# xUhEngwAng/I2V-Adapter-Unofficial

Measured on AMD Instinct MI355X. Metric: denoising steps/sec @ 16fx512x512 SD1.5+I2V-Adapter, higher is better.
Workload: dtype f16

## Files before the change

i2v-adapter-unofficial_amd/csrc/attention.hip:

```cpp
#include <cstdlib>
#include <type_traits>

#include "common.h"

namespace {

constexpr float DEFER_THR = 8.0f;

__device__ __forceinline__ float fast_exp2(float x) { return __builtin_amdgcn_exp2f(x); }
__device__ __forceinline__ float max3(float a, float b, float c) { return fmaxf(fmaxf(a, b), c); }

__device__ __forceinline__ float xor16_max(float x) { return lane_xor16_max(x); }
__device__ __forceinline__ float xor32_max(float x) { return lane_xor32_max(x); }

__device__ __forceinline__ uint32_t pack_rtz(float a, float b) {
  const auto h = __builtin_amdgcn_cvt_pkrtz(a, b);
  return __builtin_bit_cast(uint32_t, h);
}
__device__ __forceinline__ uint32_t pack_rn(float a, float b) {
  const f16x2 h = {(f16)a, (f16)b};
  return __builtin_bit_cast(uint32_t, h);
}

#ifndef I2V_ATTN_XCD_REMAP
#define I2V_ATTN_XCD_REMAP 1
#endif
#ifndef I2V_ATTN_OCC_D80
#define I2V_ATTN_OCC_D80 1
#endif
template <int DQK, int DPV, int QT, int KVT, bool SPARE, bool WALK = false>
__global__ __launch_bounds__(256)
__attribute__((amdgpu_waves_per_eu(DQK == 64 && DPV == 48 && QT == 2 && KVT == 64 && !WALK ? 4 : (DQK == 96 && DPV == 80 && !WALK ? I2V_ATTN_OCC_D80 : 1))))
void attn_kernel(const i2v_attn_params p, const float scale_log2, const int qbw_arg) {
  const int qbw = WALK ? qbw_arg : 1;
  constexpr int KS = DQK + 8;
  constexpr int VS = KVT + 8;
  constexpr int KSTEPS = DQK / 32;
  constexpr int DT = DPV / 16;
  constexpr int NKT = KVT / 16;
  constexpr int NS2 = KVT / 32;
  constexpr int KCH = DQK / 8;
  constexpr int VCH = KVT / 8;
  static_assert((KVT * KCH) % 256 == 0, "the K tile must be whole 16-byte chunks per thread");
  constexpr int NKC = (KVT * KCH) / 256;
  constexpr int NVC = (DPV * VCH + 255) / 256;
  constexpr int NSTG = WALK ? 1 : 2;
  __shared__ __attribute__((aligned(16))) f16 sKb[NSTG][KVT * KS];
  __shared__ __attribute__((aligned(16))) f16 sVb[NSTG][DPV * VS];

  const int tid = threadIdx.x, lane = tid & 63, wave = tid >> 6;
  const int g = lane >> 4, l15 = lane & 15;
  int qb = blockIdx.x, h = blockIdx.y, bq = blockIdx.z;
  {
    const int nqb = gridDim.x, pairs = gridDim.y * gridDim.z;
    if (I2V_ATTN_XCD_REMAP && p.lk <= 128 && (nqb * (int)gridDim.z) % 8 == 0) {
      const int lin = blockIdx.x + nqb * (blockIdx.y + gridDim.y * blockIdx.z);
      const int xcd = lin & 7, slot = lin >> 3;
      h = slot % (int)gridDim.y;
      const int unit = (slot / (int)gridDim.y) * 8 + xcd;
      qb = unit % nqb;
      bq = unit / nqb;
    } else if (I2V_ATTN_XCD_REMAP && pairs % 8 == 0) {
      const int lin = blockIdx.x + nqb * (blockIdx.y + gridDim.y * blockIdx.z);
      const int xcd = lin & 7, slot = lin >> 3;
      const int pair = (slot / nqb) * 8 + xcd;
      qb = slot % nqb;
      h = pair % (int)gridDim.y;
      bq = pair / (int)gridDim.y;
    }
  }
  const int bkv = bq / p.kv_group;
  const int d = p.head_dim, lq = p.lq, lk = p.lk;
  const int qb_first = qb * qbw;
  int q0 = qb_first * (64 * QT) + wave * (16 * QT);

  const f16* __restrict__ Q = reinterpret_cast<const f16*>(p.q) + (int64_t)bq * p.q_batch_stride + h * d;
  const f16* __restrict__ Kg = reinterpret_cast<const f16*>(p.k) + (int64_t)bkv * p.k_batch_stride + h * d;
  const f16* __restrict__ Vg =
      reinterpret_cast<const f16*>(p.vt) + (int64_t)bkv * p.vt_batch_stride + (int64_t)h * d * p.vt_row_stride;

  f16x8 qf[QT][KSTEPS];
  f32x4 o[DT][QT];
  f32x4 negm[QT];
  float lrow[QT];
  f16x8 qraw[QT][KSTEPS];
  auto fetch_q = [&](int q0f) {
#pragma unroll
    for (int qt = 0; qt < QT; ++qt) {
      const int row = q0f + qt * 16 + l15;
#pragma unroll
      for (int s = 0; s < KSTEPS; ++s) {
        const int dd = 32 * s + 8 * g;
        qraw[qt][s] = (row < lq && dd < d) ? ld_global_16B(Q + (int64_t)row * p.q_row_stride + dd) : zero8();
      }
    }
  };
  auto load_q = [&]() {
#pragma unroll
    for (int qt = 0; qt < QT; ++qt) {
#pragma unroll
      for (int s = 0; s < KSTEPS; ++s) {
        f16x8 v = qraw[qt][s];
#pragma unroll
        for (int e = 0; e < 8; ++e) v[e] = (f16)((float)v[e] * scale_log2);
        qf[qt][s] = v;
      }
    }
#pragma unroll
    for (int i = 0; i < DT; ++i)
#pragma unroll
      for (int j = 0; j < QT; ++j) o[i][j] = f32x4{0.f, 0.f, 0.f, 0.f};
#pragma unroll
    for (int j = 0; j < QT; ++j) {
      negm[j] = f32x4{0.f, 0.f, 0.f, 0.f};
      lrow[j] = 0.f;
    }
  };
  fetch_q(q0);

  constexpr int OOB = 0x40000000;
  f16x8 rk[NKC], rv[NVC];
  int k_off[NKC], v_off[NVC], k_lds[NKC], v_lds[NVC];
  const auto k_rsrc = __builtin_amdgcn_make_buffer_rsrc(
      const_cast<f16*>(Kg), 0, (int)(((int64_t)(lk - 1) * p.k_row_stride + d) * 2), 0x00020000);
  const auto v_rsrc = __builtin_amdgcn_make_buffer_rsrc(
      const_cast<f16*>(Vg), 0, (int)(((int64_t)(d - 1) * p.vt_row_stride + ((lk + 7) & ~7)) * 2), 0x00020000);
#pragma unroll
  for (int i = 0; i < NKC; ++i) {
    const int id = tid + 256 * i;
    const int row = id / KCH, c = id - row * KCH;
    k_off[i] = 8 * c < d ? (int)((row * p.k_row_stride + 8 * c) * 2) : OOB;
    const int lrow = (row & ~28) | ((row & 4) << 2) | ((row & 24) >> 1);
    k_lds[i] = lrow * KS + 8 * c;
  }
#pragma unroll
  for (int i = 0; i < NVC; ++i) {
    const int id = tid + 256 * i;
    const int row = id / VCH, c = id - row * VCH;
    v_off[i] = row < d ? (int)((row * p.vt_row_stride + 8 * c) * 2) : OOB;
    const bool real = row < DPV && !(SPARE && row == d);
    v_lds[i] = real ? row * VS + 8 * c : (tid % DPV) * VS + KVT;
  }
  if (SPARE && tid < NSTG * VCH) {
    f16x8 ones;
#pragma unroll
    for (int e = 0; e < 8; ++e) ones[e] = (f16)1.f;
    *reinterpret_cast<f16x8*>(&sVb[tid / VCH][d * VS + 8 * (tid % VCH)]) = ones;
  }
  const int k_tile_bytes = (int)(KVT * p.k_row_stride * 2);

  auto issue = [&](int t) {
    const int ks = t * k_tile_bytes, vs = t * (KVT * 2);
#pragma unroll
    for (int i = 0; i < NKC; ++i)
      rk[i] = __builtin_bit_cast(f16x8, __builtin_amdgcn_raw_buffer_load_b128(k_rsrc, k_off[i], ks, 0));
#pragma unroll
    for (int i = 0; i < NVC; ++i)
      rv[i] = __builtin_bit_cast(f16x8, __builtin_amdgcn_raw_buffer_load_b128(v_rsrc, v_off[i], vs, 0));
  };
  auto mask_tail_v = [&](int t) {
#pragma unroll
    for (int i = 0; i < NVC; ++i) {
      const int key0 = t * KVT + 8 * ((tid + 256 * i) % VCH);
#pragma unroll
      for (int e = 0; e < 8; ++e)
        if (key0 + e >= lk) rv[i][e] = (f16)0.f;
    }
  };
  auto commit = [&](int stage) {
    f16* sK = sKb[stage];
    f16* sV = sVb[stage];
#pragma unroll
    for (int i = 0; i < NKC; ++i) *reinterpret_cast<f16x8*>(&sK[k_lds[i]]) = rk[i];
#pragma unroll
    for (int i = 0; i < NVC; ++i) *reinterpret_cast<f16x8*>(&sV[v_lds[i]]) = rv[i];
  };

  const int ntiles = (lk + KVT - 1) / KVT;
  const bool partial = (lk % KVT) != 0;
  issue(0);
  if (ntiles == 1 && partial) mask_tail_v(0);
  commit(0);
  __syncthreads();

  auto process = [&](auto tail_c, auto more_c, const int t) {
    constexpr bool TAIL = decltype(tail_c)::value;
    constexpr bool more = decltype(more_c)::value;
    if (more) issue(t + 1);
    const f16* sK = sKb[t & 1];
    const f16* sV = sVb[t & 1];

    f32x4 sacc[NKT][QT];
#ifdef I2V_SETPRIO
    __builtin_amdgcn_s_setprio(1);
#endif
#pragma unroll
    for (int kt = 0; kt < NKT; ++kt) {
      const int krow = 16 * kt + l15;
#pragma unroll
      for (int s = 0; s < KSTEPS; ++s) {
        const f16x8 kf = *reinterpret_cast<const f16x8*>(&sK[krow * KS + 32 * s + 8 * g]);
#pragma unroll
        for (int j = 0; j < QT; ++j) sacc[kt][j] = mfma16x16x32(kf, qf[j][s], s == 0 ? negm[j] : sacc[kt][j]);
      }
    }

#ifdef I2V_SETPRIO
    __builtin_amdgcn_s_setprio(0);
#endif
    const int key_base = t * KVT;
    const bool first = t == 0;
    f16x8 pf[QT][NS2];
#pragma unroll
    for (int j = 0; j < QT; ++j) {
      float sv[NKT][4];
#pragma unroll
      for (int kt = 0; kt < NKT; ++kt)
#pragma unroll
        for (int r = 0; r < 4; ++r) {
          float v = sacc[kt][j][r];
          if (TAIL) {
            const int key = key_base + 32 * (kt >> 1) + 8 * g + 4 * (kt & 1) + r;
            if (key >= lk) v = -INFINITY;
          }
          sv[kt][r] = v;
        }
      float red[4 * NKT];
#pragma unroll
      for (int kt = 0; kt < NKT; ++kt)
#pragma unroll
        for (int r = 0; r < 4; ++r) red[4 * kt + r] = sv[kt][r];
      {
        int n = 4 * NKT;
#pragma unroll
        for (int level = 0; level < 5 && n > 1; ++level) {
          int m = 0;
#pragma unroll
          for (int i = 0; i + 2 < n; i += 3) red[m++] = max3(red[i], red[i + 1], red[i + 2]);
          if (n % 3 == 2) {
            red[m] = fmaxf(red[n - 2], red[n - 1]);
            ++m;
          } else if (n % 3 == 1) {
            red[m] = red[n - 1];
            ++m;
          }
          n = m;
        }
      }
      float mx = red[0];
      if (__any(first || mx > DEFER_THR)) {
        mx = xor16_max(mx);
        mx = xor32_max(mx);
        const float dlt = first ? mx : fmaxf(mx, 0.f);
        const float alpha = first ? 1.0f : fast_exp2(-dlt);
#pragma unroll
        for (int r = 0; r < 4; ++r) negm[j][r] -= dlt;
#pragma unroll
        for (int kt = 0; kt < NKT; ++kt)
#pragma unroll
          for (int r = 0; r < 4; ++r) sv[kt][r] -= dlt;
#pragma unroll
        for (int i = 0; i < DT; ++i)
#pragma unroll
          for (int r = 0; r < 4; ++r) o[i][j][r] *= alpha;
        if (!SPARE) lrow[j] *= alpha;
      }
      float ls = 0.f;
#pragma unroll
      for (int kt = 0; kt < NKT; ++kt)
#pragma unroll
        for (int r = 0; r < 4; ++r) {
          sv[kt][r] = fast_exp2(sv[kt][r]);
          if (!SPARE) ls += sv[kt][r];
        }
      if (!SPARE) lrow[j] += ls;
#pragma unroll
      for (int s2 = 0; s2 < NS2; ++s2) {
        u32x4 w;
        if (SPARE) {
          w[0] = pack_rtz(sv[2 * s2][0], sv[2 * s2][1]);
          w[1] = pack_rtz(sv[2 * s2][2], sv[2 * s2][3]);
          w[2] = pack_rtz(sv[2 * s2 + 1][0], sv[2 * s2 + 1][1]);
          w[3] = pack_rtz(sv[2 * s2 + 1][2], sv[2 * s2 + 1][3]);
        } else {
          w[0] = pack_rn(sv[2 * s2][0], sv[2 * s2][1]);
          w[1] = pack_rn(sv[2 * s2][2], sv[2 * s2][3]);
          w[2] = pack_rn(sv[2 * s2 + 1][0], sv[2 * s2 + 1][1]);
          w[3] = pack_rn(sv[2 * s2 + 1][2], sv[2 * s2 + 1][3]);
        }
        pf[j][s2] = __builtin_bit_cast(f16x8, w);
      }
    }

#ifdef I2V_SETPRIO
    __builtin_amdgcn_s_setprio(1);
#endif
#pragma unroll
    for (int s2 = 0; s2 < NS2; ++s2)
#pragma unroll
      for (int i = 0; i < DT; ++i) {
        const f16x8 vf = *reinterpret_cast<const f16x8*>(&sV[(i * 16 + l15) * VS + 32 * s2 + 8 * g]);
#pragma unroll
        for (int j = 0; j < QT; ++j) o[i][j] = mfma16x16x32(vf, pf[j][s2], o[i][j]);
      }

#ifdef I2V_SETPRIO
    __builtin_amdgcn_s_setprio(0);
#endif
    if (more) {
      if (partial && t + 2 == ntiles) mask_tail_v(t + 1);
      commit((t + 1) & 1);
      __syncthreads();
    }
  };

  for (int qi = 0; qi < qbw; ++qi) {
    if (WALK) {
      if ((qb_first + qi) * (64 * QT) >= lq) break;
      q0 = (qb_first + qi) * (64 * QT) + wave * (16 * QT);
    }
    load_q();
    if (WALK && qi + 1 < qbw) fetch_q(q0 + 64 * QT);
    for (int t = 0; t + 1 < ntiles; ++t) process(std::false_type{}, std::true_type{}, t);
    if (partial)
      process(std::true_type{}, std::false_type{}, ntiles - 1);
    else
      process(std::false_type{}, std::false_type{}, ntiles - 1);

    f16* __restrict__ O = reinterpret_cast<f16*>(p.o) + (int64_t)bq * p.o_batch_stride + h * d;
#pragma unroll
    for (int j = 0; j < QT; ++j) {
      float lt;
      if (SPARE) {
        float cand = 0.f;
#pragma unroll
        for (int i = 0; i < DT; ++i)
#pragma unroll
          for (int r = 0; r < 4; ++r)
            if (i == (d >> 4) && r == (d & 3)) cand = o[i][j][r];
        lt = __shfl(cand, (((d & 15) >> 2) << 4) | l15, 64);
      } else {
        lt = lrow[j];
        lt += __shfl_xor(lt, 16, 64);
        lt += __shfl_xor(lt, 32, 64);
      }
      const float inv = 1.0f / lt;
      const int row = q0 + j * 16 + l15;
      if (row >= lq) continue;
      if (p.lse != nullptr && g == 0)
        p.lse[((int64_t)bq * p.heads + h) * lq + row] = __builtin_amdgcn_logf(lt) - negm[j][0];
#pragma unroll
      for (int i = 0; i < DT; ++i) {
        const int dd = i * 16 + 4 * g;
        if (dd >= d) continue;
        f16* dst = O + (int64_t)row * p.o_row_stride + dd;
        f16x4 ov;
        if (p.accumulate) {
          const f16x4 prev = *reinterpret_cast<const f16x4*>(dst);
#pragma unroll
          for (int r = 0; r < 4; ++r) ov[r] = (f16)((float)prev[r] + p.acc_scale * o[i][j][r] * inv);
        } else {
#pragma unroll
          for (int r = 0; r < 4; ++r) ov[r] = (f16)(o[i][j][r] * inv);
        }
        *reinterpret_cast<f16x4*>(dst) = ov;
      }
    }
  }
}

inline bool al(const void* p, uintptr_t a) { return (reinterpret_cast<uintptr_t>(p) % a) == 0; }

template <int DQK, int DPV, bool SPARE>
int launch_q(const i2v_attn_params& p, hipStream_t s) {
  const float scale_log2 = p.scale * 1.4426950408889634f;
  int qt = 1;
  if (p.lq >= 128 && (DQK <= 96 || DQK == 160)) qt = 2;
  static const int qt_env = getenv("I2V_ATTN_QT") ? atoi(getenv("I2V_ATTN_QT")) : 0;
  static const int kvt_env = getenv("I2V_ATTN_KVT") ? atoi(getenv("I2V_ATTN_KVT")) : 0;
  if (qt_env == 1 || qt_env == 2) qt = qt_env;
  int kvt = 64;
  if (DQK == 64 && p.lk > 64 && p.lk <= 96) kvt = 96;
  if (kvt_env == 64 || (kvt_env == 128 && DQK <= 64) || (kvt_env == 96 && DQK == 64)) kvt = kvt_env;
  const dim3 block(256);
  const int nqb = (int)i2v_cdiv(p.lq, 64 * qt);
  static const int walk_off = getenv("I2V_ATTN_WALK") ? (atoi(getenv("I2V_ATTN_WALK")) == 0) : 0;
  int qbw = 1;
  if (!walk_off && p.lk <= kvt) {
    const int64_t wgs = (int64_t)nqb * p.heads * p.batch_q;
    qbw = (int)(wgs / 1024);
    if (qbw > 8) qbw = 8;
    if (qbw > nqb) qbw = nqb;
    if (qbw < 1) qbw = 1;
  }
  const bool walk = qbw > 1;
  const dim3 grid((unsigned)i2v_cdiv(nqb, qbw), (unsigned)p.heads, (unsigned)p.batch_q);
#define I2V_ATTN_LAUNCH(QTV, KVTV)                                                                                       \
  do {                                                                                                                   \
    if (walk)                                                                                                            \
      hipLaunchKernelGGL((attn_kernel<DQK, DPV, QTV, KVTV, SPARE, true>), grid, block, 0, s, p, scale_log2, qbw);        \
    else                                                                                                                 \
      hipLaunchKernelGGL((attn_kernel<DQK, DPV, QTV, KVTV, SPARE, false>), grid, block, 0, s, p, scale_log2, 1);         \
  } while (0)
  if constexpr (DQK == 64) {
    if (kvt == 96) {
      if (qt == 2) I2V_ATTN_LAUNCH(2, 96); else I2V_ATTN_LAUNCH(1, 96);
      return i2v_check_launch("i2v_attention_f16");
    }
  }
  if constexpr (DQK <= 64) {
    if (kvt == 128) {
      if (qt == 2) I2V_ATTN_LAUNCH(2, 128); else I2V_ATTN_LAUNCH(1, 128);
      return i2v_check_launch("i2v_attention_f16");
    }
  }
  if (qt == 2) I2V_ATTN_LAUNCH(2, 64); else I2V_ATTN_LAUNCH(1, 64);
#undef I2V_ATTN_LAUNCH
  return i2v_check_launch("i2v_attention_f16");
}

template <int DQK, int DPV>
int launch_d(const i2v_attn_params& p, hipStream_t s) {
  return p.head_dim < DPV ? launch_q<DQK, DPV, true>(p, s) : launch_q<DQK, DPV, false>(p, s);
}

}

#ifdef I2V_VARIANTS
int i2v_attention32_try(const i2v_attn_params& p, hipStream_t s);
int i2v_attention_pipe_try(const i2v_attn_params& p, hipStream_t s);
#endif

extern "C" int i2v_attention_f16(const i2v_attn_params* pp, i2v_stream_t stream) {
  I2V_CHECK_ARG(pp != nullptr, "i2v_attention_f16: null params");
  const i2v_attn_params& p = *pp;
  I2V_CHECK_ARG(p.q && p.k && p.vt && p.o, "i2v_attention_f16: null pointer");
  I2V_CHECK_ARG(p.batch_q > 0 && p.kv_group > 0 && p.batch_q % p.kv_group == 0,
                "i2v_attention_f16: batch_q (%d) must be a positive multiple of kv_group (%d)", p.batch_q, p.kv_group);
  I2V_CHECK_ARG(p.heads > 0 && p.lq > 0 && p.lk > 0, "i2v_attention_f16: heads, lq, lk must be positive");
  I2V_CHECK_ARG(!(p.lse != nullptr && p.accumulate), "i2v_attention_f16: lse output is not combined with accumulate");
  I2V_CHECK_ARG(p.head_dim > 0 && p.head_dim % 8 == 0 && p.head_dim <= 160,
                "i2v_attention_f16: head_dim (%d) must be a multiple of 8 and <= 160", p.head_dim);
  I2V_CHECK_ARG(p.q_row_stride % 8 == 0 && p.k_row_stride % 8 == 0 && p.q_batch_stride % 8 == 0 &&
                    p.k_batch_stride % 8 == 0,
                "i2v_attention_f16: q / k strides must be multiples of 8 elements");
  I2V_CHECK_ARG(p.vt_row_stride % 8 == 0 && p.vt_batch_stride % 8 == 0 && p.vt_row_stride >= ((p.lk + 7) / 8) * 8,
                "i2v_attention_f16: vt_row_stride must be a multiple of 8 and >= lk rounded up to 8");
  I2V_CHECK_ARG(p.o_row_stride % 4 == 0 && p.o_batch_stride % 4 == 0, "i2v_attention_f16: o strides must be multiples of 4");
  I2V_CHECK_ARG(al(p.q, 16) && al(p.k, 16) && al(p.vt, 16) && al(p.o, 8), "i2v_attention_f16: pointer alignment");
  I2V_CHECK_ARG(p.heads <= 65535 && p.batch_q <= 65535, "i2v_attention_f16: heads / batch_q exceed the grid limits");
  I2V_CHECK_ARG(p.k_row_stride > 0 && ((int64_t)p.lk + 128) * p.k_row_stride * 2 < (1ll << 30) &&
                    p.vt_row_stride > 0 && ((int64_t)p.head_dim * p.vt_row_stride + 256) * 2 < (1ll << 30),
                "i2v_attention_f16: one (batch, head) slice of K / V^T must span less than 1 GiB");
  hipStream_t s = reinterpret_cast<hipStream_t>(stream);
  const int d = p.head_dim;
  if (d <= 16) return launch_d<32, 16>(p, s);
  if (d <= 32) return launch_d<32, 32>(p, s);
#ifdef I2V_VARIANTS
  if (d > 32 && d < 48) {
    const int rc = i2v_attention_pipe_try(p, s);
    if (rc != 0) return rc < 0 ? rc : I2V_OK;
  }
  if (d > 32 && d <= 48) {
    const int rc = i2v_attention32_try(p, s);
    if (rc != 0) return rc < 0 ? rc : I2V_OK;
  }
#endif
  if (d <= 48) return launch_d<64, 48>(p, s);
  if (d <= 64) return launch_d<64, 64>(p, s);
  if (d <= 80) return launch_d<96, 80>(p, s);
  if (d <= 96) return launch_d<96, 96>(p, s);
  if (d <= 128) return launch_d<128, 128>(p, s);
  return launch_d<160, 160>(p, s);
}
```

Measured before the change: 20.99.

## Add max-free attention path fixing max from diagonal tile, with fallback redo

Adds a MAXFREE attention variant. It computes the row max once from a first tile (the diagonal tile when lq==lk) and then skips all later max tracking and rescaling. Row sums are accumulated with an MFMA against a ones vector instead of scalar adds. If any final row sum overflows a threshold, the block redoes the standard online-softmax walk, which costs extra work in rare cases and adds a shared-memory flag and a barrier. The variant is on by default for selected head-dim classes via an env var and also changes the occupancy hint.

```diff
diff --git a/i2v-adapter-unofficial_amd/csrc/attention.hip b/i2v-adapter-unofficial_amd/csrc/attention.hip
--- a/i2v-adapter-unofficial_amd/csrc/attention.hip
+++ b/i2v-adapter-unofficial_amd/csrc/attention.hip
@@ -28,11 +28,12 @@
 #ifndef I2V_ATTN_OCC_D80
 #define I2V_ATTN_OCC_D80 1
 #endif
-template <int DQK, int DPV, int QT, int KVT, bool SPARE, bool WALK = false>
+template <int DQK, int DPV, int QT, int KVT, bool SPARE, bool WALK = false, bool MAXFREE = false>
 __global__ __launch_bounds__(256)
-__attribute__((amdgpu_waves_per_eu(DQK == 64 && DPV == 48 && QT == 2 && KVT == 64 && !WALK ? 4 : (DQK == 96 && DPV == 80 && !WALK ? I2V_ATTN_OCC_D80 : 1))))
-void attn_kernel(const i2v_attn_params p, const float scale_log2, const int qbw_arg) {
-  const int qbw = WALK ? qbw_arg : 1;
+__attribute__((amdgpu_waves_per_eu(DQK == 64 && DPV == 48 && QT == 2 && KVT == 64 && !WALK ? 4 : (DQK == 96 && DPV == 80 && !WALK ? (MAXFREE && QT == 2 ? 2 : I2V_ATTN_OCC_D80) : 1))))
+void attn_kernel(const i2v_attn_params p, const float scale_log2, const int aux) {
+  static_assert(!(WALK && MAXFREE), "the single-tile walk has no later tiles");
+  const int qbw = WALK ? aux : 1;
   constexpr int KS = DQK + 8;
   constexpr int VS = KVT + 8;
   constexpr int KSTEPS = DQK / 32;
@@ -83,6 +84,8 @@
   f32x4 o[DT][QT];
   f32x4 negm[QT];
   float lrow[QT];
+  f32x4 lacc[QT];
+  bool l_in_mfma = false;
   f16x8 qraw[QT][KSTEPS];
   auto fetch_q = [&](int q0f) {
 #pragma unroll
@@ -106,6 +109,8 @@
         qf[qt][s] = v;
       }
     }
+  };
+  auto reset_acc = [&]() {
 #pragma unroll
     for (int i = 0; i < DT; ++i)
 #pragma unroll
@@ -114,6 +119,7 @@
     for (int j = 0; j < QT; ++j) {
       negm[j] = f32x4{0.f, 0.f, 0.f, 0.f};
       lrow[j] = 0.f;
+      lacc[j] = f32x4{0.f, 0.f, 0.f, 0.f};
     }
   };
   fetch_q(q0);
@@ -178,17 +184,28 @@
 
   const int ntiles = (lk + KVT - 1) / KVT;
   const bool partial = (lk % KVT) != 0;
-  issue(0);
+  __shared__ int s_redo;
+  const bool fast = MAXFREE && ntiles > 1;
+  const int nfull = partial ? ntiles - 1 : ntiles;
+  int t_start = 0;
+  if (fast && lq == lk && p.kv_group == 1) {
+    t_start = (qb * (64 * QT)) / KVT;
+    if (t_start >= nfull) t_start = nfull - 1;
+  }
+  if (MAXFREE && tid == 0) s_redo = 0;
+  issue(t_start);
   if (ntiles == 1 && partial) mask_tail_v(0);
   commit(0);
   __syncthreads();
 
-  auto process = [&](auto tail_c, auto more_c, const int t) {
+  auto process = [&](auto tail_c, auto more_c, auto mode_c, const int t, const int tn, const int stage) {
     constexpr bool TAIL = decltype(tail_c)::value;
     constexpr bool more = decltype(more_c)::value;
-    if (more) issue(t + 1);
-    const f16* sK = sKb[t & 1];
-    const f16* sV = sVb[t & 1];
+    constexpr int MODE = decltype(mode_c)::value;
+    if (more) issue(tn);
+    if constexpr (MODE != 0) __builtin_amdgcn_sched_barrier(0);
+    const f16* sK = sKb[stage];
+    const f16* sV = sVb[stage];
 
     f32x4 sacc[NKT][QT];
 #ifdef I2V_SETPRIO
@@ -225,6 +242,7 @@
           }
           sv[kt][r] = v;
         }
+      if constexpr (MODE != 2) {
       float red[4 * NKT];
 #pragma unroll
       for (int kt = 0; kt < NKT; ++kt)
@@ -248,7 +266,16 @@
         }
       }
       float mx = red[0];
-      if (__any(first || mx > DEFER_THR)) {
+      if constexpr (MODE == 1) {
+        mx = xor16_max(mx);
+        mx = xor32_max(mx);
+#pragma unroll
+        for (int r = 0; r < 4; ++r) negm[j][r] = -mx;
+#pragma unroll
+        for (int kt = 0; kt < NKT; ++kt)
+#pragma unroll
+          for (int r = 0; r < 4; ++r) sv[kt][r] -= mx;
+      } else if (__any(first || mx > DEFER_THR)) {
         mx = xor16_max(mx);
         mx = xor32_max(mx);
         const float dlt = first ? mx : fmaxf(mx, 0.f);
@@ -265,15 +292,16 @@
           for (int r = 0; r < 4; ++r) o[i][j][r] *= alpha;
         if (!SPARE) lrow[j] *= alpha;
       }
+      }
       float ls = 0.f;
 #pragma unroll
       for (int kt = 0; kt < NKT; ++kt)
 #pragma unroll
         for (int r = 0; r < 4; ++r) {
           sv[kt][r] = fast_exp2(sv[kt][r]);
-          if (!SPARE) ls += sv[kt][r];
-        }
-      if (!SPARE) lrow[j] += ls;
+          if (!SPARE && MODE == 0) ls += sv[kt][r];
+        }
+      if (!SPARE && MODE == 0) lrow[j] += ls;
 #pragma unroll
       for (int s2 = 0; s2 < NS2; ++s2) {
         u32x4 w;
@@ -303,15 +331,46 @@
 #pragma unroll
         for (int j = 0; j < QT; ++j) o[i][j] = mfma16x16x32(vf, pf[j][s2], o[i][j]);
       }
+    if constexpr (!SPARE && MODE != 0) {
+      f16x8 ones;
+#pragma unroll
+      for (int e = 0; e < 8; ++e) ones[e] = (f16)1.f;
+#pragma unroll
+      for (int s2 = 0; s2 < NS2; ++s2)
+#pragma unroll
+        for (int j = 0; j < QT; ++j) lacc[j] = mfma16x16x32(ones, pf[j][s2], lacc[j]);
+    }
 
 #ifdef I2V_SETPRIO
     __builtin_amdgcn_s_setprio(0);
 #endif
     if (more) {
-      if (partial && t + 2 == ntiles) mask_tail_v(t + 1);
-      commit((t + 1) & 1);
+      if (partial && tn + 1 == ntiles) mask_tail_v(tn);
+      commit(stage ^ 1);
       __syncthreads();
     }
+  };
+  [[maybe_unused]] constexpr std::integral_constant<int, 0> mode_defer{};
+  [[maybe_unused]] constexpr std::integral_constant<int, 1> mode_first{};
+  [[maybe_unused]] constexpr std::integral_constant<int, 2> mode_free{};
+  auto row_sum = [&](const int j) {
+    float lt;
+    if (SPARE) {
+      float cand = 0.f;
+#pragma unroll
+      for (int i = 0; i < DT; ++i)
+#pragma unroll
+        for (int r = 0; r < 4; ++r)
+          if (i == (d >> 4) && r == (d & 3)) cand = o[i][j][r];
+      lt = __shfl(cand, (((d & 15) >> 2) << 4) | l15, 64);
+    } else if (MAXFREE && l_in_mfma) {
+      lt = lacc[j][0];
+    } else {
+      lt = lrow[j];
+      lt += __shfl_xor(lt, 16, 64);
+      lt += __shfl_xor(lt, 32, 64);
+    }
+    return lt;
   };
 
   for (int qi = 0; qi < qbw; ++qi) {
@@ -320,30 +379,52 @@
       q0 = (qb_first + qi) * (64 * QT) + wave * (16 * QT);
     }
     load_q();
+    reset_acc();
     if (WALK && qi + 1 < qbw) fetch_q(q0 + 64 * QT);
-    for (int t = 0; t + 1 < ntiles; ++t) process(std::false_type{}, std::true_type{}, t);
-    if (partial)
-      process(std::true_type{}, std::false_type{}, ntiles - 1);
-    else
-      process(std::false_type{}, std::false_type{}, ntiles - 1);
+    bool defer_walk = true;
+    if constexpr (MAXFREE) {
+      if (fast) {
+        auto next_tile = [&](const int i) { return i + 1 < nfull ? (i < t_start ? i : i + 1) : nfull; };
+        l_in_mfma = !SPARE;
+        int t = t_start, tn = next_tile(0);
+        process(std::false_type{}, std::true_type{}, mode_first, t, tn, 0);
+        t = tn;
+        for (int i = 1; i + 1 < ntiles; ++i) {
+          tn = next_tile(i);
+          process(std::false_type{}, std::true_type{}, mode_free, t, tn, i & 1);
+          t = tn;
+        }
+        if (partial)
+          process(std::true_type{}, std::false_type{}, mode_free, t, 0, (ntiles - 1) & 1);
+        else
+          process(std::false_type{}, std::false_type{}, mode_free, t, 0, (ntiles - 1) & 1);
+        bool bad = aux != 0;
+#pragma unroll
+        for (int j = 0; j < QT; ++j) bad |= (__float_as_uint(row_sum(j)) & 0x7fffffffu) >= 0x47000000u;
+        if (bad) s_redo = 1;
+        __syncthreads();
+        defer_walk = s_redo != 0;
+        if (defer_walk) {
+          l_in_mfma = false;
+          reset_acc();
+          issue(0);
+          commit(0);
+          __syncthreads();
+        }
+      }
+    }
+    if (defer_walk) {
+      for (int t = 0; t + 1 < ntiles; ++t) process(std::false_type{}, std::true_type{}, mode_defer, t, t + 1, t & 1);
+      if (partial)
+        process(std::true_type{}, std::false_type{}, mode_defer, ntiles - 1, 0, (ntiles - 1) & 1);
+      else
+        process(std::false_type{}, std::false_type{}, mode_defer, ntiles - 1, 0, (ntiles - 1) & 1);
+    }
 
     f16* __restrict__ O = reinterpret_cast<f16*>(p.o) + (int64_t)bq * p.o_batch_stride + h * d;
 #pragma unroll
     for (int j = 0; j < QT; ++j) {
-      float lt;
-      if (SPARE) {
-        float cand = 0.f;
-#pragma unroll
-        for (int i = 0; i < DT; ++i)
-#pragma unroll
-          for (int r = 0; r < 4; ++r)
-            if (i == (d >> 4) && r == (d & 3)) cand = o[i][j][r];
-        lt = __shfl(cand, (((d & 15) >> 2) << 4) | l15, 64);
-      } else {
-        lt = lrow[j];
-        lt += __shfl_xor(lt, 16, 64);
-        lt += __shfl_xor(lt, 32, 64);
-      }
+      const float lt = row_sum(j);
       const float inv = 1.0f / lt;
       const int row = q0 + j * 16 + l15;
       if (row >= lq) continue;
@@ -411,6 +492,17 @@
   if constexpr (DQK <= 64) {
     if (kvt == 128) {
       if (qt == 2) I2V_ATTN_LAUNCH(2, 128); else I2V_ATTN_LAUNCH(1, 128);
+      return i2v_check_launch("i2v_attention_f16");
+    }
+  }
+  static const int maxfree = getenv("I2V_ATTN_MAXFREE") ? atoi(getenv("I2V_ATTN_MAXFREE")) : 1;
+  constexpr bool MAXFREE_CLASS = (DQK == 64 && DPV == 48 && SPARE) || (DQK == 96 && DPV == 80 && !SPARE) || (DQK == 160 && DPV == 160 && !SPARE);
+  if constexpr (MAXFREE_CLASS) {
+    if ((maxfree == 2 || maxfree == 3 || (maxfree == 1 && DQK != 160)) && !walk && p.lk > 64) {
+      if (qt == 2)
+        hipLaunchKernelGGL((attn_kernel<DQK, DPV, 2, 64, SPARE, false, true>), grid, block, 0, s, p, scale_log2, maxfree == 2);
+      else
+        hipLaunchKernelGGL((attn_kernel<DQK, DPV, 1, 64, SPARE, false, true>), grid, block, 0, s, p, scale_log2, maxfree == 2);
       return i2v_check_launch("i2v_attention_f16");
     }
   }
```

Result: no change. 21.09, median of 6 (+0.5%).
